# BadgerTechnologies/navigation

Measured on AMD Instinct MI355X. Metric: scored trajectories/sec (whole node) + costmap inflation cells/sec, 400x400 map, higher is better.
Workload: dtype f64

## Files before the change

### navigation_amd/csrc/planner_score.h

```cpp
#pragma once
#include "planner_common.h"

namespace navgpu {

__host__ __device__ inline size_t score_bits_bytes(int win) {
  return (((size_t)4 * win * ((win + 31) >> 5) * 4) + 15) & ~(size_t)15;
}
__host__ __device__ inline size_t score_scratch_bytes(int win) { return score_bits_bytes(win); }
__device__ __forceinline__ int divSmall(int n, int d) {
  int q = (int)((float)n * __builtin_amdgcn_rcpf((float)d));
  int r = n - q * d;
  if (r < 0) {
    --q;
    r += d;
  }
  if (r >= d) ++q;
  return q;
}

struct WorldToMapFast {
  const Geom& g;
  const double& inv_res;
  __device__ __forceinline__ bool operator()(double wx, double wy, uint32_t& mx, uint32_t& my) const {
    const double dx = wx - g.ox, dy = wy - g.oy;
    const double qx = dx * inv_res, qy = dy * inv_res;
    double fx = floor(qx), fy = floor(qy);
    const double rx = qx - fx, ry = qy - fy;
    if (__builtin_expect(fmin(rx, ry) < 1.0e-7 || fmax(rx, ry) > 1.0 - 1.0e-7, 0)) {
      fx = !(dx >= 0.0) ? -1.0 : (qx >= 1.0e6 ? 1.0e6 : (double)(int)(dx / g.res));
      fy = !(dy >= 0.0) ? -1.0 : (qy >= 1.0e6 ? 1.0e6 : (double)(int)(dy / g.res));
    }
    int ix, iy;
    asm("v_cvt_i32_f64 %0, %1" : "=v"(ix) : "v"(fx));
    asm("v_cvt_i32_f64 %0, %1" : "=v"(iy) : "v"(fy));
    mx = (uint32_t)ix;
    my = (uint32_t)iy;
    return mx < g.nx && my < g.ny;
  }
};

__device__ __forceinline__ void addCritic(double& total, bool en, double value, double scale) {
  if (!en) return;
  double cost = value;
  if (cost != 0) cost *= scale;
  total += cost;
}

constexpr uint32_t kScoreAuxBytes = 64;
__host__ __device__ inline uint32_t score_prep_reject_bytes(const PlannerDev& pl) { return (pl.max_axis * pl.max_axis + 255u) & ~255u; }
__host__ __device__ inline uint32_t score_prep_reject_offset(const PlannerDev& pl) { return pl.prep_stride - score_prep_reject_bytes(pl); }
template <size_t kAllowAbove = 48 * 1024, typename... P, typename... A>
void launchScore(void (*kernel)(P...), dim3 grid, int threads, size_t lds, hipStream_t s, A... args) {
  if (lds > kAllowAbove) hipFuncSetAttribute((const void*)kernel, hipFuncAttributeMaxDynamicSharedMemorySize, (int)lds);
  hipLaunchKernelGGL(kernel, grid, dim3(threads), lds, s, args...);
}
size_t score_table_row_bytes(const PlannerDev& pl);
size_t score_table_lds_bytes(const PlannerDev& pl);
bool score_sweep_applies(const PlannerDev& pl);
uint32_t launch_score_sweep(const PlannerDev& pl, uint32_t first, uint32_t count, hipStream_t s);
uint32_t launch_score_sweep_list(const PlannerDev& pl, const uint32_t* list, uint32_t count, hipStream_t s);

}
```

### navigation_amd/csrc/planner_score.hip

```cpp
#include "planner_score.h"

namespace navgpu {

#ifdef NAVGPU_PREP_TIMING
__device__ unsigned long long g_prep_stats[16];
#define PREP_STAMP(i) prep_t[i] = wall_clock64()
#else
#define PREP_STAMP(i)
#endif

struct ScoreRobot {
  uint32_t inst;
  Geom g;
  navgpu_robot_state st;
  const uint8_t* master;
  const uint32_t *dpath, *dgoal, *dfront;
  const int32_t* cnt;
  uint32_t nfp;
  int win, wx0, wy0;
  int win_bytes, nw;
};
__device__ __forceinline__ ScoreRobot scoreRobot(const PlannerDev& pl, uint32_t inst) {
  ScoreRobot r;
  r.inst = inst;
  r.g = geomOf(pl, inst);
  r.st = pl.state[inst];
  r.master = pl.master + (size_t)inst * pl.cells_padded;
  r.dpath = pl.path + (size_t)inst * pl.cells;
  r.dgoal = pl.goal + (size_t)inst * pl.cells;
  r.dfront = pl.goal_front + (size_t)inst * pl.cells;
  r.cnt = pl.axis_count + 4 * inst;
  r.nfp = pl.fp_n[inst];
  r.win = (int)pl.win;
  r.win_bytes = (r.win * r.win + 15) & ~15;
  r.nw = (r.win + 31) >> 5;
  return r;
}
__device__ __forceinline__ void placeWindow(ScoreRobot& r) {
  double fx = floor(((double)r.st.pos[0] - r.g.ox) / r.g.res), fy = floor(((double)r.st.pos[1] - r.g.oy) / r.g.res);
  fx = fmin(fmax(fx, -1.0e6), 1.0e6);
  fy = fmin(fmax(fy, -1.0e6), 1.0e6);
  r.wx0 = (int)fx - r.win / 2;
  r.wy0 = (int)fy - r.win / 2;
}

template <bool EXPLICIT>
__device__ __forceinline__ void stageInputs(const PlannerDev& pl, ScoreRobot& r, double* s_fp, float (*s_axis)[kMaxAxis], int* s_cnt, uint8_t* s_win) {
  const uint32_t tid = threadIdx.x;
  const Geom& g = r.g;
  if (tid < 2 * r.nfp) s_fp[tid] = pl.fp_spec[(size_t)r.inst * kMaxFootprint * 2 + tid];
  if (!EXPLICIT) {
    for (uint32_t i = tid; i < 3 * kMaxAxis; i += blockDim.x) {
      uint32_t a = i / kMaxAxis, k = i - a * kMaxAxis;
// ... 130 lines not shown
  const navgpu_robot_state& st = r.st;
  const uint32_t nfp = r.nfp;
  const int K = (int)pl.tab_steps;
  const int tnfp = (int)pl.tab_nfp;
  const int nth_s = r.cnt[2];
  const int lrows = (int)pl.tab_nth;
  double* s_trig = reinterpret_cast<double*>(s_dyn + r.win_bytes + score_bits_bytes(r.win));
  double* s_rot = s_trig + (size_t)lrows * K * 4;
  float* s_th = reinterpret_cast<float*>(s_rot + (size_t)lrows * K * tnfp * 2);
  __syncthreads();
  const double dt_t = c.sim_time / K;
  if ((int)tid < nth_s) {
    float pth = st.pos[2];
    const float vth = s_axis[2][tid];
    for (int k = 0; k < K; ++k) {
      s_th[tid * K + k] = pth;
      pth = (float)(pth + vth * dt_t);
    }
  }
  __syncthreads();
  for (int e = tid; e < nth_s * K; e += blockDim.x) {
    const double th = s_th[e];
    double sn, cs, sn2, cs2;
    sincos(th, &sn, &cs);
    sincos(M_PI_2 + th, &sn2, &cs2);
    s_trig[4 * e] = cs;
    s_trig[4 * e + 1] = sn;
    s_trig[4 * e + 2] = cs2;
    s_trig[4 * e + 3] = sn2;
    for (int v = 0; v < (int)nfp && v < tnfp; ++v) {
      const double sx = s_fp[2 * v], sy = s_fp[2 * v + 1];
      s_rot[(e * tnfp + v) * 2] = sx * cs - sy * sn;
      s_rot[(e * tnfp + v) * 2 + 1] = sx * sn + sy * cs;
    }
  }
}

__device__ __forceinline__ void storeImage(const PlannerDev& pl, const ScoreRobot& r, const uint8_t* s_dyn) {
  uint4* img = reinterpret_cast<uint4*>(pl.prep + (size_t)r.inst * pl.prep_stride);
  const uint4* lds = reinterpret_cast<const uint4*>(s_dyn);
  const uint32_t n16 = pl.prep_bytes >> 4;
  for (uint32_t i = threadIdx.x; i < n16; i += blockDim.x) img[i] = lds[i];
}

__device__ __forceinline__ void storeSweepScalars(const PlannerDev& pl, const ScoreRobot& r, const float (*s_axis)[kMaxAxis], int* s_cnt,
                                                  const uint8_t* s_dyn) {
  const uint32_t tid = threadIdx.x;
  const navgpu_dwa_config& c = pl.cfg;
  const Geom& g = r.g;
  const int32_t* cnt = r.cnt;
  const uint32_t inst = r.inst;
  const int win = r.win, wx0 = r.wx0, wy0 = r.wy0, nw = r.nw;
  const uint32_t* s_fb = reinterpret_cast<const uint32_t*>(s_dyn + r.win_bytes);
  uint8_t* rej = pl.prep + (size_t)inst * pl.prep_stride + score_prep_reject_offset(pl);
  int32_t* aux = reinterpret_cast<int32_t*>(rej - kScoreAuxBytes);
  const int c0 = win / 2;
  const uint32_t w_c0 = (uint32_t)(c0 * nw + (c0 >> 5));
  const int start_fail = ((s_fb[4 * w_c0 + 2] >> (c0 & 31)) & 1u) ? 4 : (((s_fb[4 * w_c0 + 3] >> (c0 & 31)) & 1u) ? 5 : 0);
  if (tid == 0) s_cnt[0] = (win / 2) * (win / 2);
  __syncthreads();
  {
    int dmin = win * win;
    for (int it = tid; it < win * nw; it += blockDim.x) {
      const int y = it / nw, j = it - y * nw;
      uint32_t m = (c.sum_scores ? s_fb[4 * it] : s_fb[4 * it + 1]) | (start_fail == 4 ? 0u : s_fb[4 * it + 2]) | (start_fail != 0 ? 0u : s_fb[4 * it + 3]);
      const int dy = y > c0 ? y - c0 : c0 - y;
      const int p = c0 - 32 * j;
      const uint32_t right = p <= 0 ? m : (p >= 32 ? 0u : m & (0xFFFFFFFFu << p)), left = m & ~right;
      if (right) dmin = min(dmin, (32 * j + __ffs(right) - 1 - c0) * (32 * j + __ffs(right) - 1 - c0) + dy * dy);
      if (left) dmin = min(dmin, (c0 - (32 * j + 31 - __clz(left))) * (c0 - (32 * j + 31 - __clz(left))) + dy * dy);
    }
    atomicMin(&s_cnt[0], dmin);
  }
  __syncthreads();
  if (tid == 0) {
    const double inv_res = pl.inv_res, fpd = c.forward_point_distance;
    const bool en_fwd = pl.scale_goal != 0 || (pl.align_on[inst] && pl.scale_path != 0);
    const uint32_t fwd_margin = (uint32_t)fmin(ceil(fabs(fpd) * inv_res) + 1.0, 1.0e6);
    const bool fwd_screen = !en_fwd || (2u * fwd_margin < g.nx && 2u * fwd_margin < g.ny);
    const uint32_t fwd_lo = en_fwd ? fwd_margin : 0u, fwd_nx = g.nx - 2u * fwd_lo, fwd_ny = g.ny - 2u * fwd_lo;
    const bool need_margin = !((uint32_t)wx0 - fwd_lo < fwd_nx && (uint32_t)(wx0 + win - 1) - fwd_lo < fwd_nx && (uint32_t)wy0 - fwd_lo < fwd_ny &&
                               (uint32_t)(wy0 + win - 1) - fwd_lo < fwd_ny);
    aux[0] = wx0;
    aux[1] = wy0;
    aux[2] = (int32_t)fwd_lo;
    aux[3] = (int32_t)fwd_nx;
    aux[4] = (int32_t)fwd_ny;
    aux[5] = need_margin ? 1 : 0;
    aux[6] = fwd_screen ? 1 : 0;
    aux[7] = (int)floor(sqrt((double)s_cnt[0]));
    aux[8] = start_fail;
  }
  const int nyv = max(cnt[1], 1), nxyv = cnt[0] * cnt[1];
  for (int i = tid; i < nxyv; i += blockDim.x) {
    const int ix = i / nyv, iy = i - ix * nyv;
    const double vmag = hyp2((double)s_axis[0][ix], (double)s_axis[1][iy]);
    const double eps = 1e-4;
    rej[i] = (uint8_t)(((c.min_trans_vel >= 0 && vmag + eps < c.min_trans_vel) ? 1 : 0) | ((c.max_trans_vel >= 0 && vmag - eps > c.max_trans_vel) ? 2 : 0));
  }
}

struct ScoreInputs {
  static constexpr int kAxisChunks = (3 * kMaxAxis + kScoreThreads - 1) / kScoreThreads;
  double fp;
  float axis[kAxisChunks];
};
__device__ __forceinline__ ScoreInputs loadInputs(const PlannerDev& pl, const ScoreRobot& r) {
  const uint32_t tid = threadIdx.x;
  ScoreInputs in;
  in.fp = pl.fp_spec[(size_t)r.inst * kMaxFootprint * 2 + (tid < 2 * r.nfp ? tid : 0)];
#pragma unroll
  for (int u = 0; u < ScoreInputs::kAxisChunks; ++u) {
    const uint32_t i = min(tid + (uint32_t)u * kScoreThreads, 3u * kMaxAxis - 1), a = i / kMaxAxis, k = i - a * kMaxAxis;
    in.axis[u] = pl.axis_samples[((size_t)r.inst * 3 + a) * pl.max_axis + min(k, pl.max_axis - 1)];
    if (k >= pl.max_axis) in.axis[u] = 0.f;
  }
  return in;
}
__device__ __forceinline__ void loadImage(const PlannerDev& pl, const ScoreRobot& r, const ScoreInputs& in, double* s_fp, float (*s_axis)[kMaxAxis],
                                          uint8_t* s_dyn) {
  const uint32_t tid = threadIdx.x;
  const uint4* img = reinterpret_cast<const uint4*>(pl.prep + (size_t)r.inst * pl.prep_stride);
  uint4* lds = reinterpret_cast<uint4*>(s_dyn);
  const uint32_t n16 = pl.prep_bytes >> 4;
  for (uint32_t i = tid; i < n16; i += blockDim.x) lds[i] = img[i];
  if (tid < 2 * r.nfp) s_fp[tid] = in.fp;
#pragma unroll
  for (int u = 0; u < ScoreInputs::kAxisChunks; ++u) {
    const uint32_t i = tid + (uint32_t)u * kScoreThreads;
    if (i < 3u * kMaxAxis) s_axis[i / kMaxAxis][i % kMaxAxis] = in.axis[u];
  }
  __syncthreads();
}

template <bool EXPLICIT, int CHUNK, bool AGG, bool TERMS = false, bool PROBES = false>
__device__ __forceinline__ void scoreSamples(const PlannerDev& pl, const ScoreRobot& r, const double* s_fp, const float (*s_axis)[kMaxAxis],
                                             const uint8_t* s_dyn, double* s_rc, int* s_ri, int* s_cnt, const float* explicit_sample,
                                             SampleTerms* terms = nullptr, uint32_t n_probes = 0, double* probe_cost = nullptr) {
  static_assert(!PROBES || (EXPLICIT && !TERMS), "probes are explicit samples");
  const uint32_t tid = threadIdx.x;
  const navgpu_dwa_config& c = pl.cfg;
  const Geom& g = r.g;
  const navgpu_robot_state& st = r.st;
  const uint8_t* master = r.master;
  const uint32_t *dpath = r.dpath, *dgoal = r.dgoal, *dfront = r.dfront;
  const int32_t* cnt = r.cnt;
  const uint32_t inst = r.inst, nfp = r.nfp;
  const int n_samples = PROBES ? (int)n_probes : EXPLICIT ? 1 : cnt[3];
  const int win = r.win, wx0 = r.wx0, wy0 = r.wy0, win_bytes = r.win_bytes, nw = r.nw;
  const uint8_t* s_win = s_dyn;
  const bool walk_swap = pl.cfg.allow_unknown != 0;
// ... 536 lines not shown
__global__ __launch_bounds__(kScoreThreads) void k_score_explicit_agg(PlannerDev pl, uint32_t first, const float* explicit_sample) {
  scoreExplicit<true>(pl, first, explicit_sample);
}
template <bool AGG>
__device__ __forceinline__ void checkTraj(const PlannerDev& pl, const ProbeBatch& pb) {
  extern __shared__ __align__(16) uint8_t s_dyn[];
  __shared__ double s_fp[2 * kMaxFootprint];
  __shared__ float s_axis[3][kMaxAxis];
  __shared__ int s_cnt[2];
  const uint32_t p0 = pb.offsets[blockIdx.y], n = pb.offsets[blockIdx.y + 1] - p0;
  if (blockIdx.x * kScoreThreads >= n) return;
  ScoreRobot r = scoreRobot(pl, pb.instances[blockIdx.y]);
  if (blockIdx.x == 0 && threadIdx.x == 0) pl.osc_flags[r.inst] = 0;
  stageInputs<true>(pl, r, s_fp, s_axis, s_cnt, s_dyn);
  __syncthreads();
  buildScreens(pl, r, s_dyn, reinterpret_cast<uint32_t*>(s_dyn + r.win_bytes + score_bits_bytes(r.win)));
  __syncthreads();
  scoreSamples<true, 12, AGG, false, true>(pl, r, s_fp, s_axis, s_dyn, nullptr, nullptr, s_cnt, pb.vel + 3 * (size_t)p0, nullptr, n, pb.cost + p0);
}
__global__ __launch_bounds__(kScoreThreads) void k_check_traj(PlannerDev pl, ProbeBatch pb) { checkTraj<false>(pl, pb); }
__global__ __launch_bounds__(kScoreThreads) void k_check_traj_agg(PlannerDev pl, ProbeBatch pb) { checkTraj<true>(pl, pb); }

__global__ __launch_bounds__(kScoreThreads) void k_score_terms(PlannerDev pl, uint32_t inst, SampleTerms* terms) {
  scoreGen<16, false, true>(pl, RobotRange{inst}, terms);
}
__global__ __launch_bounds__(kScoreThreads) void k_score_terms_agg(PlannerDev pl, uint32_t inst, SampleTerms* terms) {
  scoreGen<16, true, true>(pl, RobotRange{inst}, terms);
}

size_t score_window_bytes(uint32_t win) {
  return (((size_t)win * win + 15) & ~(size_t)15) + score_bits_bytes((int)win);
}
size_t score_table_row_bytes(const PlannerDev& pl) { return (size_t)pl.tab_steps * ((4 + 2 * pl.tab_nfp) * sizeof(double) + sizeof(float)); }
size_t score_table_bytes(const PlannerDev& pl) {
  return ((size_t)pl.tab_nth * score_table_row_bytes(pl) + 15) & ~(size_t)15;
}
size_t score_table_lds_bytes(const PlannerDev& pl) {
  return ((size_t)pl.tab_rows * score_table_row_bytes(pl) + 15) & ~(size_t)15;
}
uint32_t score_table_rows(const PlannerDev& pl, uint32_t win) {
  const size_t wb = score_window_bytes(win), row = score_table_row_bytes(pl);
  if (row == 0 || wb + score_table_bytes(pl) + score_scratch_bytes((int)win) > 150u * 1024u) return 0;
  for (size_t budget : {(size_t)NAVGPU_SCORE_TAB_LDS_KB * 1024, (size_t)52 * 1024, (size_t)78 * 1024}) {
    if (wb + 16 >= budget) continue;
    const size_t r = (budget - wb - 16) / row;
    if (r >= 1) return (uint32_t)std::min<size_t>(r, pl.tab_nth);
  }
  return 0;
}
size_t score_prep_bytes(const PlannerDev& pl) {
  return score_window_bytes(pl.win) + (pl.use_tables ? score_table_bytes(pl) : 0);
}
size_t score_prep_slot_bytes(const PlannerDev& pl) {
  return ((score_prep_bytes(pl) + 255) & ~(size_t)255) + kScoreAuxBytes + score_prep_reject_bytes(pl);
}
static uint32_t sweepLaunch(const PlannerDev& pl, RobotRange r, uint32_t count, hipStream_t s) { return launch_score_sweep(pl, r.first, count, s); }
static uint32_t sweepLaunch(const PlannerDev& pl, RobotList r, uint32_t count, hipStream_t s) { return launch_score_sweep_list(pl, r.list, count, s); }
template <class Robots>
static uint32_t launchScoreCycle(const PlannerDev& pl_in, Robots robots, uint32_t count, hipStream_t s) {
  PlannerDev pl = pl_in;
  const size_t win_bytes = score_window_bytes(pl.win);
  const size_t scratch = score_scratch_bytes((int)pl.win);
  if (score_sweep_applies(pl)) {
    pl.tab_bytes = (uint32_t)score_table_bytes(pl);
    pl.prep_bytes = (uint32_t)score_prep_bytes(pl);
    launchScore(k_score_prep_tab<Robots>, dim3(1, count), kScorePrepThreads, win_bytes + score_table_bytes(pl) + scratch, s, pl, robots);
    return sweepLaunch(pl, robots, count, s);
  }
  pl.use_tables = 0;
  pl.prep_bytes = (uint32_t)score_prep_bytes(pl);
  const uint32_t gen_blocks = (pl.max_samples + kScoreThreads - 1) / kScoreThreads;
  launchScore(prepGenKernel(robots), dim3(1, count), kScoreThreads, win_bytes + scratch, s, pl, robots);
  auto gen = pl.mg_generic        ? k_score_gen_agg<Robots>
             : pl.fp_chunk <= 6  ? k_score_gen<6, Robots>
             : pl.fp_chunk <= 9  ? k_score_gen<9, Robots>
             : pl.fp_chunk <= 12 ? k_score_gen<12, Robots>
                                 : k_score_gen<16, Robots>;
  launchScore(gen, dim3(gen_blocks, count), kScoreThreads, win_bytes, s, pl, robots, (const float*)nullptr);
  return gen_blocks;
}
uint32_t launch_score(const PlannerDev& pl, uint32_t first, uint32_t count, const float* explicit_sample, hipStream_t s) {
  if (explicit_sample) {
    const size_t lds = score_window_bytes(pl.win) + score_scratch_bytes((int)pl.win);
    launchScore(pl.mg_generic ? k_score_explicit_agg : k_score_explicit, dim3(1, count), kScoreThreads, lds, s, pl, first, explicit_sample);
    return 1;
  }
  return launchScoreCycle(pl, RobotRange{first}, count, s);
}
uint32_t launch_score_list(const PlannerDev& pl, const uint32_t* list, uint32_t count, hipStream_t s) { return launchScoreCycle(pl, RobotList{list}, count, s); }

void launch_check_traj(const PlannerDev& pl, const ProbeBatch& pb, uint32_t n_robots, uint32_t max_probes, hipStream_t s) {
  const size_t lds = score_window_bytes(pl.win) + score_scratch_bytes((int)pl.win);
  launchScore(pl.mg_generic ? k_check_traj_agg : k_check_traj, dim3((max_probes + kScoreThreads - 1) / kScoreThreads, n_robots), kScoreThreads, lds, s, pl, pb);
}

void launch_score_terms(const PlannerDev& pl_in, uint32_t inst, SampleTerms* terms, hipStream_t s) {
  PlannerDev pl = pl_in;
  const size_t win_bytes = score_window_bytes(pl.win);
  pl.use_tables = 0;
  pl.prep_bytes = (uint32_t)score_prep_bytes(pl);
  const uint32_t gen_blocks = (pl.max_samples + kScoreThreads - 1) / kScoreThreads;
  launchScore(k_score_prep_gen, dim3(1, 1), kScoreThreads, win_bytes + score_scratch_bytes((int)pl.win), s, pl, RobotRange{inst});
  launchScore(pl.mg_generic ? k_score_terms_agg : k_score_terms, dim3(gen_blocks, 1), kScoreThreads, win_bytes, s, pl, inst, terms);
}

#ifdef NAVGPU_PREP_TIMING
extern "C" int navgpu_debug_prep_stats(unsigned long long* out16, int reset) {
  if (out16) hipMemcpyFromSymbol(out16, HIP_SYMBOL(g_prep_stats), sizeof(unsigned long long) * 16);
  if (reset) {
    unsigned long long z[16] = {0};
    hipMemcpyToSymbol(HIP_SYMBOL(g_prep_stats), z, sizeof(z));
  }
  return 0;
}
#endif

}
```

### navigation_amd/csrc/planner_score_sweep.hip

```cpp
#include "planner_score.h"

namespace navgpu {

constexpr int kSweepThreads = NAVGPU_SCORE_TAB_THREADS;
constexpr int kSweepWaves = 6;
#ifndef NAVGPU_SWEEP_BLOCK_STEPS
#define NAVGPU_SWEEP_BLOCK_STEPS 4
#endif
#ifndef NAVGPU_SWEEP_QUEUE
#define NAVGPU_SWEEP_QUEUE 768
#endif
constexpr int kSweepBlockSteps = NAVGPU_SWEEP_BLOCK_STEPS;
constexpr int kSweepQueue = NAVGPU_SWEEP_QUEUE;
constexpr uint32_t kWalkFailed = 0x80000000u;
#ifdef NAVGPU_SWEEP_COUNTS
__device__ unsigned long long g_sweep_counts[16];
#define SW_COUNT(slot_, n_)                                                                    \
  do {                                                                                           \
    const unsigned long long swc_ = (unsigned long long)(n_);                                    \
    if ((threadIdx.x & 63u) == 0) atomicAdd(&g_sweep_counts[slot_], swc_);                       \
  } while (0)
#else
#define SW_COUNT(slot_, n_)
#endif
#ifdef NAVGPU_SWEEP_TIMING
__device__ unsigned long long g_sweep_stats[16];
#define SW_STAMP(v) const unsigned long long v = __builtin_amdgcn_s_memtime()
#define SW_ACC(i, x) sw_t[i] += (x)
#else
#define SW_STAMP(v)
#define SW_ACC(i, x)
#endif

template <int CHUNK, bool TRIGF, bool KEEP, class Robots>
__global__ __launch_bounds__(kSweepThreads, kSweepWaves) void k_score_sweep(PlannerDev pl, Robots robots) {
  constexpr int THREADS = kSweepThreads;
  extern __shared__ __align__(16) uint8_t s_dyn[];
  uint8_t* s_win = s_dyn;
  __shared__ double s_rc[THREADS / 64];
  __shared__ int s_ri[THREADS / 64];
  __shared__ int s_cnt[2];
  __shared__ float s_qx[kSweepQueue], s_qy[kSweepQueue];
  __shared__ uint32_t s_qt[kSweepQueue];
  __shared__ uint32_t s_obs[THREADS];
  __shared__ uint32_t s_qn[2];
  __shared__ uint32_t s_more[3];

  const uint32_t inst = robots(blockIdx.z);
  const uint32_t tid = threadIdx.x;
#ifdef NAVGPU_SWEEP_TIMING
  unsigned long long sw_t[10] = {0, 0, 0, 0, 0, 0, 0, 0, 0, 0};
#endif
  SW_STAMP(sw0);
  __builtin_amdgcn_s_setprio(3);
  const navgpu_dwa_config& c = pl.cfg;
  const Geom g = geomOf(pl, inst);
  const navgpu_robot_state st = pl.state[inst];
  const uint8_t* master = pl.master + (size_t)inst * pl.cells_padded;
  const uint32_t* dpath = pl.path + (size_t)inst * pl.cells;
  const uint32_t* dgoal = pl.goal + (size_t)inst * pl.cells;
  const uint32_t* dfront = pl.goal_front + (size_t)inst * pl.cells;
  const int32_t* cnt = pl.axis_count + 4 * inst;
  const int n_samples = cnt[3];
  const uint32_t nfp = pl.fp_n[inst];
  const int win = (int)pl.win;

  if (tid == 0) s_cnt[0] = s_cnt[1] = 0;
  if (tid < 2) s_qn[tid] = 0;
  if (tid < 3) s_more[tid] = 0;
  s_obs[tid] = 0;
  const uint8_t* rej_bytes = pl.prep + (size_t)inst * pl.prep_stride + score_prep_reject_offset(pl);
  const int32_t* aux = reinterpret_cast<const int32_t*>(rej_bytes - kScoreAuxBytes);
  const int wx0 = aux[0], wy0 = aux[1];
  const uint32_t fwd_lo = (uint32_t)aux[2], fwd_nx = (uint32_t)aux[3], fwd_ny = (uint32_t)aux[4];
  const bool need_margin = aux[5] != 0, fwd_screen = aux[6] != 0;
  const int free_cells = aux[7];
  const int start_fail = aux[8];
  const uint32_t osc = pl.osc_flags[inst];
  const int32_t align_on = pl.align_on[inst];
  const int win_bytes = (win * win + 15) & ~15;
  const int nw = (win + 31) >> 5;
  const bool walk_swap = pl.cfg.allow_unknown != 0;
  const uint32_t walk_fail = walk_swap ? 255u : 254u;
  const int K = (int)pl.tab_steps;
  const int tnfp = (int)pl.tab_nfp;
  const int lrows = (int)pl.tab_rows;
  double* s_trig = reinterpret_cast<double*>(s_dyn + win_bytes + score_bits_bytes(win));
  double* s_rot = s_trig + (size_t)lrows * K * 4;
  const int nxy = max(cnt[0] * cnt[1], 1);
  const uint32_t part_slot = blockIdx.y * gridDim.x + blockIdx.x;
  const int t_row_base = (int)blockIdx.y * (int)pl.tab_rows;
  const int t_rows = min(max(cnt[2] - t_row_base, 0), (int)pl.tab_rows);
  const int t_li0 = (int)blockIdx.x * THREADS;
  if (t_li0 >= t_rows * nxy) {
    if (tid == 0) {
      pl.part_cost[(size_t)inst * pl.score_blocks + part_slot] = 1.0e300;
      pl.part_index[(size_t)inst * pl.score_blocks + part_slot] = 0x7FFFFFFF;
    }
    return;
  }
  const int li = t_li0 + (int)tid;
  const int t_row = divSmall(li, nxy);
  const int t_r = li - t_row * nxy;
  const int t_ith = t_row_base + t_row;
  const bool in_range = n_samples > 0 && t_row < t_rows;
  const int sidx = t_r * cnt[2] + t_ith;
  const int nyv = max(cnt[1], 1);
  const int s_ix = divSmall(t_r, nyv), s_iy = t_r - s_ix * nyv;
  const float* axis = pl.axis_samples + (size_t)inst * 3 * pl.max_axis;
  const uint32_t amax = pl.max_axis - 1u;
  const float vs0 = axis[min((uint32_t)s_ix, amax)], vs1 = axis[pl.max_axis + min((uint32_t)s_iy, amax)], vs2 = axis[2u * pl.max_axis + min((uint32_t)t_ith, amax)];
  const uint32_t rej_xy = rej_bytes[in_range ? t_r : 0];
  auto rejected = [&]() { return !in_range || ((rej_xy & 1u) && (c.min_rot_vel >= 0 && fabs((double)vs2) + 1e-4 < c.min_rot_vel)) || (rej_xy & 2u) || K <= 0; };
  if constexpr (!KEEP) {
    if (start_fail != 0) {
      const unsigned long long m_acc = __ballot(!rejected());
      if ((tid & 63u) == 0 && m_acc != 0ull) atomicAdd(&pl.counters[2 * inst], __popcll(m_acc));
      if (tid == 0) {
        pl.part_cost[(size_t)inst * pl.score_blocks + part_slot] = 1.0e300;
        pl.part_index[(size_t)inst * pl.score_blocks + part_slot] = 0x7FFFFFFF;
      }
      return;
    }
  }
  {
    const uint4* img = reinterpret_cast<const uint4*>(pl.prep + (size_t)inst * pl.prep_stride);
    uint4* lds = reinterpret_cast<uint4*>(s_dyn);
    const int last = max(t_rows, 1) - 1;
    const int r0 = min(divSmall(t_li0, nxy), last);
    const int r1 = min(divSmall(t_li0 + THREADS - 1, nxy), last);
    const int n16w = (int)((win_bytes + score_bits_bytes(win)) >> 4);
    const int ncopy = r1 - r0 + 1;
    const int n_trig = ncopy * K * 2, n_rot = ncopy * K * tnfp;
    const int l_trig = n16w + r0 * K * 2, g_trig = n16w + (t_row_base + r0) * K * 2;
    const int l_rot = n16w + lrows * K * 2 + r0 * K * tnfp, g_rot = n16w + (int)pl.tab_nth * K * 2 + (t_row_base + r0) * K * tnfp;
    const int ia0 = (int)tid, ia1 = (int)tid + THREADS;
    const uint4 va0 = img[min(ia0, n16w - 1)], va1 = img[min(ia1, n16w - 1)];
    const uint4 vb = img[g_trig + min((int)tid, n_trig - 1)], vc = img[g_rot + min((int)tid, max(n_rot, 1) - 1)];
    if (ia0 < n16w) lds[ia0] = va0;
    if (ia1 < n16w) lds[ia1] = va1;
    if ((int)tid < n_trig) lds[l_trig + (int)tid] = vb;
    if ((int)tid < n_rot) lds[l_rot + (int)tid] = vc;
    if (n16w > 2 * THREADS || n_trig > THREADS || n_rot > THREADS) {
      for (int i = (int)tid + 2 * THREADS; i < n16w; i += THREADS) lds[i] = img[i];
      for (int i = (int)tid + THREADS; i < n_trig; i += THREADS) lds[l_trig + i] = img[g_trig + i];
      for (int i = (int)tid + THREADS; i < n_rot; i += THREADS) lds[l_rot + i] = img[g_rot + i];
    }
  }
  SW_STAMP(sw1a);
  __syncthreads();
  __builtin_amdgcn_s_setprio(0);
  SW_STAMP(sw1);
  SW_ACC(0, sw1a - sw0);
  SW_ACC(1, sw1 - sw1a);

  auto inWin = [&](int x, int y) { return (unsigned)(x - wx0) < (unsigned)win && (unsigned)(y - wy0) < (unsigned)win; };
  auto cellCost = [&](int x, int y) -> uint8_t {
    const bool in = inWin(x, y);
    uint32_t v = s_win[in ? (y - wy0) * win + (x - wx0) : 0];
    asm volatile("" : "+v"(v));
    if (walk_swap && v >= 254u) v ^= 1u;
    if (__builtin_expect(!in, 0)) v = master[y * g.nx + x];
    return (uint8_t)v;
  };
  const double inv_res = pl.inv_res;
  const WorldToMapFast w2m{g, inv_res};

  auto walkWindow = [&](const double x, const double y, const int te, uint32_t& mx, bool& outside) -> bool {
    const double* rot = s_rot + (size_t)te * tnfp * 2;
    bool off = false;
    outside = false;
    mx = 0;
    uint32_t ux, uy;
    off |= !w2m(x + rot[0], y + rot[1], ux, uy);
    const int fx0 = (int)ux, fy0 = (int)uy;
    int pxc = fx0, pyc = fy0;
    for (uint32_t v = 1; v <= nfp; ++v) {
      int vx = fx0, vy = fy0;
      if (v < nfp) {
        off |= !w2m(x + rot[2 * v], y + rot[2 * v + 1], ux, uy);
        vx = (int)ux;
        vy = (int)uy;
// ... 35 lines not shown
    w2m(x + rot[0], y + rot[1], ux, uy);
    const int fx0 = (int)ux, fy0 = (int)uy;
    int pxc = fx0, pyc = fy0;
    for (uint32_t v = 1; v <= nfp; ++v) {
      int vx = fx0, vy = fy0;
      if (v < nfp) {
        w2m(x + rot[2 * v], y + rot[2 * v + 1], ux, uy);
        vx = (int)ux;
        vy = (int)uy;
      }
      int deltax = vx - pxc, deltay = vy - pyc;
      deltax = deltax < 0 ? -deltax : deltax;
      deltay = deltay < 0 ? -deltay : deltay;
      int lx = pxc, ly = pyc;
      int xinc1, xinc2, yinc1, yinc2, den, num, numadd, numpixels;
      xinc1 = xinc2 = (vx >= pxc) ? 1 : -1;
      yinc1 = yinc2 = (vy >= pyc) ? 1 : -1;
      if (deltax >= deltay) {
        xinc1 = 0;
        yinc2 = 0;
        den = deltax;
        num = deltax / 2;
        numadd = deltay;
        numpixels = deltax;
      } else {
        xinc2 = 0;
        yinc1 = 0;
        den = deltay;
        num = deltay / 2;
        numadd = deltax;
        numpixels = deltay;
      }
      for (int cp = 0; cp <= numpixels; ++cp) {
        const uint32_t cc = master[ly * g.nx + lx];
        const uint32_t ct = (walk_swap && cc >= 254u) ? (cc ^ 1u) : cc;
        mx = ct > mx ? ct : mx;
        num += numadd;
        if (num >= den) {
          num -= den;
          lx += xinc1;
          ly += yinc1;
        }
        lx += xinc2;
        ly += yinc2;
      }
      pxc = vx;
      pyc = vy;
    }
    return mx;
  };

  double total = -1.0;
  int status = NAVGPU_SAMPLE_REJECTED;
  const float vs[3] = {vs0, vs1, vs2};
  const bool reject = rejected();
  if (in_range && !reject) status = NAVGPU_SAMPLE_SCORED;
  const double dt = pl.tab_dt;
  const double xv = vs[0], yv = vs[1], thv = vs[2];
  const bool osc_fail = ((osc & NAVGPU_OSC_FORWARD_POS_ONLY) && xv < 0.0) || ((osc & NAVGPU_OSC_FORWARD_NEG_ONLY) && xv > 0.0) ||
                        ((osc & NAVGPU_OSC_STRAFE_POS_ONLY) && yv < 0.0) || ((osc & NAVGPU_OSC_STRAFE_NEG_ONLY) && yv > 0.0) ||
                        ((osc & NAVGPU_OSC_ROT_POS_ONLY) && thv < 0.0) || ((osc & NAVGPU_OSC_ROT_NEG_ONLY) && thv > 0.0);
  const double sc_obs = pl.scale_obstacle, sc_gf = pl.scale_goal, sc_al = align_on ? pl.scale_path : 0.0, sc_path = pl.scale_path,
               sc_goal = pl.scale_goal;
  const bool en_obs = sc_obs != 0, en_gf = sc_gf != 0, en_al = sc_al != 0, en_path = sc_path != 0, en_goal = sc_goal != 0;
  int first_fail = 6;
  int fail_code = 0;
  uint32_t d_gf = 0, d_al = 0, d_path = 0, d_goal = 0;
  uint32_t fail_cell = 0xFFFFFFFFu, last_c = 0, last_f = 0xFFFFFFFFu;
  const double fpd = c.forward_point_distance;
  const uint32_t N_obst = pl.cells, N_unreach = pl.cells + 1;
  if (en_obs && nfp == 0) {
    fail_code = -9;
    first_fail = 1;
  }
  const int min_order_keep = en_obs ? 1 : en_gf ? 2 : en_al ? 3 : en_path ? 4 : en_goal ? 5 : 6;
  const int min_order = KEEP ? min_order_keep : (min_order_keep < 6 ? 5 : 6);
  uint32_t fb_off = (uint32_t)win_bytes;
  asm volatile("" : "+v"(fb_off));
  const uint4* s_fb4 = reinterpret_cast<const uint4*>(s_dyn + fb_off);
  const bool scr_sum = c.sum_scores != 0;
  const bool screen_on = fwd_screen && (nfp >= 3 || !en_obs);
  float px = st.pos[0], py = st.pos[1];
  int step = 0;
  uint32_t alive_m = (in_range && !reject && !osc_fail && first_fail > min_order) ? 0xFFFFFFFFu : 0u;
#ifdef NAVGPU_SWEEP_X_NOSTEPS
  alive_m = 0;
#endif
  const bool margin_on = __builtin_amdgcn_readfirstlane((int)need_margin) != 0;
  const uint32_t lane = tid & 63u;
  const int te0 = t_row * K;
  const double vxd = vs[0], vyd = vs[1];
  uint32_t scr_z = 0xFFFFFFFFu, scr_w = 0xFFFFFFFFu;
  const uint32_t scr_off = screen_on ? 0u : 0xFFFFFFFFu;
  SW_STAMP(sw2);
  SW_ACC(2, sw2 - sw1);
  int k_free = 0;
  {
    const float spd = sqrtf(vs0 * vs0 + vs1 * vs1) * (float)(dt * inv_res) * 1.0001f + 1.0e-4f;
    int kl = K - 1;
    if (alive_m != 0u) kl = (screen_on && !margin_on && free_cells >= 3) ? (int)fminf((float)(free_cells - 2) / spd, (float)(K - 1)) : 0;
    for (int off = 32; off > 0; off >>= 1) kl = min(kl, __shfl_xor(kl, off));
    k_free = __builtin_amdgcn_readfirstlane(kl);
  }
  for (int k = 0; k < k_free; ++k) {
    const int te = te0 + k;
    const double cs = s_trig[4 * te], sn = s_trig[4 * te + 1], cs2 = s_trig[4 * te + 2], sn2 = s_trig[4 * te + 3];
    const double tx = TRIGF ? (double)(vs[0] * (float)cs) : vxd * cs, ty = TRIGF ? (double)(vs[0] * (float)sn) : vxd * sn;
    const float nxp = (float)(px + (tx + vyd * cs2) * dt);
    const float nyp = (float)(py + (ty + vyd * sn2) * dt);
    px = nxp;
    py = nyp;
  }
  if (alive_m != 0u) step = k_free;
  SW_COUNT(9, k_free);
  SW_COUNT(10, (unsigned)k_free * (unsigned)__popcll(__ballot(alive_m != 0u)));
  if constexpr (KEEP) {
    if (k_free > 0 && start_fail != 0 && alive_m != 0u) {
      first_fail = start_fail;
      fail_code = 0;
      fail_cell = (uint32_t)(wy0 + win / 2) * g.nx + (uint32_t)(wx0 + win / 2);
      scr_z = first_fail > 4 ? 0xFFFFFFFFu : 0u;
      scr_w = 0u;
      alive_m = first_fail > min_order ? 0xFFFFFFFFu : 0u;
    }
  }
  for (uint32_t blk = 0;; ++blk) {
    SW_STAMP(sb0);
    if (__ballot(alive_m != 0u) != 0ull) {
      for (int it = 0; it < kSweepBlockSteps; ++it) {
        const int sc = min(step, K - 1);
        const int te = te0 + sc;
        const double x = px, y = py;
        const double cs = s_trig[4 * te], sn = s_trig[4 * te + 1];
        SW_COUNT(4, 1);
        SW_COUNT(8, __popcll(__ballot(alive_m != 0u)));
        const double cs2 = s_trig[4 * te + 2], sn2 = s_trig[4 * te + 3];
        const double tx = TRIGF ? (double)(vs[0] * (float)cs) : vxd * cs, ty = TRIGF ? (double)(vs[0] * (float)sn) : vxd * sn;
        const float nxp = (float)(px + (tx + vyd * cs2) * dt);
        const float nyp = (float)(py + (ty + vyd * sn2) * dt);
        uint32_t cx, cy;
        const bool ok_c = w2m(x, y, cx, cy);
        const uint32_t lx = cx - (uint32_t)wx0, ly = cy - (uint32_t)wy0;
        bool in_w = max(lx, ly) < (uint32_t)win;
        uint32_t force = (sc == K - 1) ? 0xFFFFFFFFu : scr_off;
        if (margin_on) {
          in_w = in_w && ok_c;
          if (!((cx - fwd_lo < fwd_nx) && (cy - fwd_lo < fwd_ny))) force = 0xFFFFFFFFu;
        }
        const uint32_t fb_i = in_w ? ly * (uint32_t)nw + (lx >> 5) : 0u;
        const uint4 fbw = s_fb4[fb_i];
        const uint32_t any = (scr_sum ? fbw.x : fbw.y) | (fbw.z & scr_z) | (fbw.w & scr_w) | force | (in_w ? 0u : 0xFFFFFFFFu);
        const bool unscr = ((any >> (lx & 31u)) & alive_m & 1u) != 0u;
        px = nxp;
        py = nyp;
        step -= (int)alive_m;
// ... 156 lines not shown
      if ((tid & 63u) == (uint32_t)(__ffsll((long long)__ballot(true)) - 1)) atomicAdd(&g_sweep_counts[7], 1ull);
#endif
      if (off || mx_cost >= walk_fail) {
        atomicOr(&s_obs[owner], kWalkFailed);
      } else if (tag >> 31) {
        const double f_cost = (walk_swap && mx_cost == 254u) ? 255.0 : (double)mx_cost;
        uint32_t cx, cy;
        w2m(x, y, cx, cy);
        const double occ = fmax(fmax(0.0, f_cost), (double)cellCost(cx, cy));
        atomicAdd(&s_obs[owner], (uint32_t)occ);
      }
    }
    SW_STAMP(sb3);
    SW_ACC(6, sb3 - sb2);
    __syncthreads();
    SW_STAMP(sb4);
    SW_ACC(7, sb4 - sb3);
    if ((s_obs[tid] & kWalkFailed) != 0u && first_fail > 1) {
      fail_code = -6;
      first_fail = 1;
      alive_m = 0;
    }
    if (!more) break;
  }

  {
    const bool reached = last_f != 0xFFFFFFFFu && first_fail > 1;
    const uint32_t cmax = pl.cells - 1u;
    uint32_t v_fail = 0;
    if constexpr (KEEP) v_fail = (first_fail == 4 ? dpath : dgoal)[min(fail_cell, cmax)];
    const uint32_t v_gf = dfront[min(last_f, cmax)], v_al = dpath[min(last_f, cmax)];
    const uint32_t v_path = dpath[min(last_c, cmax)], v_goal = dgoal[min(last_c, cmax)];
    if constexpr (KEEP)
      if ((first_fail == 4 || first_fail == 5) && fail_code == 0) fail_code = v_fail == N_obst ? -3 : -2;
    if (reached) {
      if (en_gf && 2 < first_fail) d_gf = v_gf;
      if (en_al && 3 < first_fail) d_al = v_al;
      if (en_path && 4 < first_fail) {
        if (v_path == N_obst || v_path == N_unreach) {
          fail_code = v_path == N_obst ? -3 : -2;
          first_fail = 4;
        } else
          d_path = v_path;
      }
      if (en_goal && 5 < first_fail) {
        if (v_goal == N_obst || v_goal == N_unreach) {
          fail_code = v_goal == N_obst ? -3 : -2;
          first_fail = 5;
        } else
          d_goal = v_goal;
      }
    }
  }
  if (in_range && !reject) {
    if (osc_fail) {
      total = -5.0;
    } else if (first_fail < 6) {
      total = KEEP ? (double)fail_code : -1.0;
    } else {
      total = 0.0;
      addCritic(total, en_obs, (double)(s_obs[tid] & ~kWalkFailed), sc_obs);
      addCritic(total, en_gf, (double)d_gf, sc_gf);
      addCritic(total, en_al, (double)d_al, sc_al);
      addCritic(total, en_path, (double)d_path, sc_path);
      addCritic(total, en_goal, (double)d_goal, sc_goal);
    }
  }
  if constexpr (KEEP) {
    if (in_range && pl.sample_cost) {
      pl.sample_cost[(size_t)inst * pl.max_samples + sidx] = total;
      pl.sample_status[(size_t)inst * pl.max_samples + sidx] = status;
    }
  }

  const bool valid = in_range && status == NAVGPU_SAMPLE_SCORED && total >= 0.0;
  double bc = valid ? total : 1.0e300;
  int bi = valid ? sidx : 0x7FFFFFFF;
  for (int off = 32; off > 0; off >>= 1) {
    double oc = __shfl_down(bc, off);
    int oi = __shfl_down(bi, off);
    if (oc < bc || (oc == bc && oi < bi)) {
      bc = oc;
      bi = oi;
    }
  }
  const unsigned long long m_scored = __ballot(in_range && status == NAVGPU_SAMPLE_SCORED);
  const unsigned long long m_valid = __ballot(valid);
  if ((tid & 63) == 0) {
    s_rc[tid >> 6] = bc;
    s_ri[tid >> 6] = bi;
    atomicAdd(&s_cnt[0], __popcll(m_scored));
    atomicAdd(&s_cnt[1], __popcll(m_valid));
  }
  __syncthreads();
  if (tid == 0) {
    for (int w = 1; w < THREADS / 64; ++w)
      if (s_rc[w] < bc || (s_rc[w] == bc && s_ri[w] < bi)) {
        bc = s_rc[w];
        bi = s_ri[w];
      }
    pl.part_cost[(size_t)inst * pl.score_blocks + part_slot] = bc;
    pl.part_index[(size_t)inst * pl.score_blocks + part_slot] = bi;
    if (s_cnt[0]) atomicAdd(&pl.counters[2 * inst], s_cnt[0]);
    if (s_cnt[1]) atomicAdd(&pl.counters[2 * inst + 1], s_cnt[1]);
  }
#ifdef NAVGPU_SWEEP_TIMING
// ... 66 lines not shown
```

Measured before the change: 6.768 billion.

## Precompute per-pair and per-row sweep records in prep; use DPP wave-min

Prep now writes 16-byte per-(vx,vy) records holding the velocities, the free-step bound and the reject and oscillation flags, plus per-rotation-row flag records. The sweep kernel reads one uint4 instead of recomputing axis loads, the hypot and sqrt, and the oscillation tests per thread. The wave minimum uses DPP plus readlane instead of shuffles, and row/column index division is replaced by a wave-uniform base with an increment loop. This adds prep work and prep-slot memory, and the float-bit min trick relies on kl values being non-negative.

```diff
diff --git a/navigation_amd/csrc/planner_score.h b/navigation_amd/csrc/planner_score.h
--- a/navigation_amd/csrc/planner_score.h
+++ b/navigation_amd/csrc/planner_score.h
@@ -47,8 +47,24 @@
 }
 
 constexpr uint32_t kScoreAuxBytes = 64;
-__host__ __device__ inline uint32_t score_prep_reject_bytes(const PlannerDev& pl) { return (pl.max_axis * pl.max_axis + 255u) & ~255u; }
-__host__ __device__ inline uint32_t score_prep_reject_offset(const PlannerDev& pl) { return pl.prep_stride - score_prep_reject_bytes(pl); }
+struct alignas(16) SweepPair {
+  float vs0, vs1;
+  float kl_pair;
+  uint32_t flags;
+};
+struct alignas(16) SweepRow {
+  double thv;
+  float vs2;
+  uint32_t flags;
+};
+static_assert(sizeof(SweepPair) == 16 && sizeof(SweepRow) == 16, "one 16-byte load per record");
+constexpr uint32_t kPairRejMin = 1u, kPairRejMax = 2u, kPairOsc = 4u;
+constexpr uint32_t kRowRejRot = 1u, kRowOsc = 2u;
+__host__ __device__ inline uint32_t score_prep_pair_bytes(const PlannerDev& pl) { return pl.max_axis * pl.max_axis * (uint32_t)sizeof(SweepPair); }
+__host__ __device__ inline uint32_t score_prep_record_bytes(const PlannerDev& pl) {
+  return (score_prep_pair_bytes(pl) + pl.max_axis * (uint32_t)sizeof(SweepRow) + 255u) & ~255u;
+}
+__host__ __device__ inline uint32_t score_prep_record_offset(const PlannerDev& pl) { return pl.prep_stride - score_prep_record_bytes(pl); }
 template <size_t kAllowAbove = 48 * 1024, typename... P, typename... A>
 void launchScore(void (*kernel)(P...), dim3 grid, int threads, size_t lds, hipStream_t s, A... args) {
   if (lds > kAllowAbove) hipFuncSetAttribute((const void*)kernel, hipFuncAttributeMaxDynamicSharedMemorySize, (int)lds);
diff --git a/navigation_amd/csrc/planner_score.hip b/navigation_amd/csrc/planner_score.hip
--- a/navigation_amd/csrc/planner_score.hip
+++ b/navigation_amd/csrc/planner_score.hip
@@ -1,4 +1,5 @@
 #include "planner_score.h"
+#include "navgpu_fleet.h"
 
 namespace navgpu {
 
@@ -235,8 +236,8 @@
   const uint32_t inst = r.inst;
   const int win = r.win, wx0 = r.wx0, wy0 = r.wy0, nw = r.nw;
   const uint32_t* s_fb = reinterpret_cast<const uint32_t*>(s_dyn + r.win_bytes);
-  uint8_t* rej = pl.prep + (size_t)inst * pl.prep_stride + score_prep_reject_offset(pl);
-  int32_t* aux = reinterpret_cast<int32_t*>(rej - kScoreAuxBytes);
+  uint8_t* rec = pl.prep + (size_t)inst * pl.prep_stride + score_prep_record_offset(pl);
+  int32_t* aux = reinterpret_cast<int32_t*>(rec - kScoreAuxBytes);
   const int c0 = win / 2;
   const uint32_t w_c0 = (uint32_t)(c0 * nw + (c0 >> 5));
   const int start_fail = ((s_fb[4 * w_c0 + 2] >> (c0 & 31)) & 1u) ? 4 : (((s_fb[4 * w_c0 + 3] >> (c0 & 31)) & 1u) ? 5 : 0);
@@ -273,13 +274,39 @@
     aux[6] = fwd_screen ? 1 : 0;
     aux[7] = (int)floor(sqrt((double)s_cnt[0]));
     aux[8] = start_fail;
-  }
+    aux[9] = (int32_t)pl.osc_flags[inst];
+  }
+  const uint32_t osc = pl.osc_flags[inst];
+  const int free_cells = (int)floor(sqrt((double)s_cnt[0]));
+  const int K = (int)pl.tab_steps;
+  const double dt = pl.tab_dt;
+  const double eps = 1e-4;
+  SweepPair* pairs = reinterpret_cast<SweepPair*>(rec);
   const int nyv = max(cnt[1], 1), nxyv = cnt[0] * cnt[1];
   for (int i = tid; i < nxyv; i += blockDim.x) {
     const int ix = i / nyv, iy = i - ix * nyv;
-    const double vmag = hyp2((double)s_axis[0][ix], (double)s_axis[1][iy]);
-    const double eps = 1e-4;
-    rej[i] = (uint8_t)(((c.min_trans_vel >= 0 && vmag + eps < c.min_trans_vel) ? 1 : 0) | ((c.max_trans_vel >= 0 && vmag - eps > c.max_trans_vel) ? 2 : 0));
+    const float vs0 = s_axis[0][ix], vs1 = s_axis[1][iy];
+    const double xv = vs0, yv = vs1;
+    const double vmag = hyp2(xv, yv);
+    const bool osc_xy = ((osc & NAVGPU_OSC_FORWARD_POS_ONLY) && xv < 0.0) || ((osc & NAVGPU_OSC_FORWARD_NEG_ONLY) && xv > 0.0) ||
+                        ((osc & NAVGPU_OSC_STRAFE_POS_ONLY) && yv < 0.0) || ((osc & NAVGPU_OSC_STRAFE_NEG_ONLY) && yv > 0.0);
+    const float spd = sqrtf(vs0 * vs0 + vs1 * vs1) * (float)(dt * pl.inv_res) * 1.0001f + 1.0e-4f;
+    SweepPair p;
+    p.vs0 = vs0;
+    p.vs1 = vs1;
+    p.kl_pair = free_cells >= 3 ? fminf((float)(free_cells - 2) / spd, (float)(K - 1)) : 0.f;
+    p.flags = ((c.min_trans_vel >= 0 && vmag + eps < c.min_trans_vel) ? kPairRejMin : 0u) | ((c.max_trans_vel >= 0 && vmag - eps > c.max_trans_vel) ? kPairRejMax : 0u) |
+              (osc_xy ? kPairOsc : 0u);
+    pairs[i] = p;
+  }
+  SweepRow* rows = reinterpret_cast<SweepRow*>(rec + score_prep_pair_bytes(pl));
+  for (int i = tid; i < cnt[2]; i += blockDim.x) {
+    SweepRow w;
+    w.vs2 = s_axis[2][i];
+    w.thv = w.vs2;
+    w.flags = ((c.min_rot_vel >= 0 && fabs((double)w.vs2) + eps < c.min_rot_vel) ? kRowRejRot : 0u) |
+              ((((osc & NAVGPU_OSC_ROT_POS_ONLY) && w.thv < 0.0) || ((osc & NAVGPU_OSC_ROT_NEG_ONLY) && w.thv > 0.0)) ? kRowOsc : 0u);
+    rows[i] = w;
   }
 }
 
@@ -922,7 +949,7 @@
   return score_window_bytes(pl.win) + (pl.use_tables ? score_table_bytes(pl) : 0);
 }
 size_t score_prep_slot_bytes(const PlannerDev& pl) {
-  return ((score_prep_bytes(pl) + 255) & ~(size_t)255) + kScoreAuxBytes + score_prep_reject_bytes(pl);
+  return ((score_prep_bytes(pl) + 255) & ~(size_t)255) + kScoreAuxBytes + score_prep_record_bytes(pl);
 }
 static uint32_t sweepLaunch(const PlannerDev& pl, RobotRange r, uint32_t count, hipStream_t s) { return launch_score_sweep(pl, r.first, count, s); }
 static uint32_t sweepLaunch(const PlannerDev& pl, RobotList r, uint32_t count, hipStream_t s) { return launch_score_sweep_list(pl, r.list, count, s); }
@@ -974,6 +1001,20 @@
   launchScore(pl.mg_generic ? k_score_terms_agg : k_score_terms, dim3(gen_blocks, 1), kScoreThreads, win_bytes, s, pl, inst, terms);
 }
 
+extern "C" int navgpu_debug_score_setup_records(navgpu_fleet* f, uint32_t inst, int32_t* aux16, void* pairs, uint32_t n_pairs, void* rows, uint32_t n_rows) {
+  if (!f || !f->rangeOk(inst, 1) || !aux16 || (n_pairs && !pairs) || (n_rows && !rows)) return NAVGPU_ERR_INVALID;
+  FleetGuard guard_(f);
+  const PlannerDev& pl = f->pl;
+  if (!f->planner_configured || !pl.prep) return NAVGPU_ERR_STATE;
+  if (n_pairs > pl.max_axis * pl.max_axis || n_rows > pl.max_axis) return NAVGPU_ERR_CAPACITY;
+  HIP_TRY(waitStream(f->stream));
+  const uint8_t* rec = pl.prep + (size_t)inst * pl.prep_stride + score_prep_record_offset(pl);
+  HIP_TRY(hipMemcpy(aux16, rec - kScoreAuxBytes, kScoreAuxBytes, hipMemcpyDeviceToHost));
+  if (n_pairs) HIP_TRY(hipMemcpy(pairs, rec, (size_t)n_pairs * sizeof(SweepPair), hipMemcpyDeviceToHost));
+  if (n_rows) HIP_TRY(hipMemcpy(rows, rec + score_prep_pair_bytes(pl), (size_t)n_rows * sizeof(SweepRow), hipMemcpyDeviceToHost));
+  return NAVGPU_OK;
+}
+
 #ifdef NAVGPU_PREP_TIMING
 extern "C" int navgpu_debug_prep_stats(unsigned long long* out16, int reset) {
   if (out16) hipMemcpyFromSymbol(out16, HIP_SYMBOL(g_prep_stats), sizeof(unsigned long long) * 16);
diff --git a/navigation_amd/csrc/planner_score_sweep.hip b/navigation_amd/csrc/planner_score_sweep.hip
--- a/navigation_amd/csrc/planner_score_sweep.hip
+++ b/navigation_amd/csrc/planner_score_sweep.hip
@@ -31,6 +31,16 @@
 #define SW_STAMP(v)
 #define SW_ACC(i, x)
 #endif
+
+__device__ __forceinline__ uint32_t waveMinU32(uint32_t v) {
+  v = min(v, (uint32_t)__builtin_amdgcn_update_dpp((int)v, (int)v, 0xB1, 0xF, 0xF, false));
+  v = min(v, (uint32_t)__builtin_amdgcn_update_dpp((int)v, (int)v, 0x4E, 0xF, 0xF, false));
+  v = min(v, (uint32_t)__builtin_amdgcn_update_dpp((int)v, (int)v, 0x141, 0xF, 0xF, false));
+  v = min(v, (uint32_t)__builtin_amdgcn_update_dpp((int)v, (int)v, 0x140, 0xF, 0xF, false));
+  const uint32_t a = (uint32_t)__builtin_amdgcn_readlane((int)v, 0), b = (uint32_t)__builtin_amdgcn_readlane((int)v, 16);
+  const uint32_t c = (uint32_t)__builtin_amdgcn_readlane((int)v, 32), d = (uint32_t)__builtin_amdgcn_readlane((int)v, 48);
+  return min(min(a, b), min(c, d));
+}
 
 template <int CHUNK, bool TRIGF, bool KEEP, class Robots>
 __global__ __launch_bounds__(kSweepThreads, kSweepWaves) void k_score_sweep(PlannerDev pl, Robots robots) {
@@ -69,15 +79,13 @@
   if (tid < 2) s_qn[tid] = 0;
   if (tid < 3) s_more[tid] = 0;
   s_obs[tid] = 0;
-  const uint8_t* rej_bytes = pl.prep + (size_t)inst * pl.prep_stride + score_prep_reject_offset(pl);
-  const int32_t* aux = reinterpret_cast<const int32_t*>(rej_bytes - kScoreAuxBytes);
+  const uint8_t* rec_bytes = pl.prep + (size_t)inst * pl.prep_stride + score_prep_record_offset(pl);
+  const int32_t* aux = reinterpret_cast<const int32_t*>(rec_bytes - kScoreAuxBytes);
   const int wx0 = aux[0], wy0 = aux[1];
   const uint32_t fwd_lo = (uint32_t)aux[2], fwd_nx = (uint32_t)aux[3], fwd_ny = (uint32_t)aux[4];
   const bool need_margin = aux[5] != 0, fwd_screen = aux[6] != 0;
-  const int free_cells = aux[7];
   const int start_fail = aux[8];
-  const uint32_t osc = pl.osc_flags[inst];
-  const int32_t align_on = pl.align_on[inst];
+  const int32_t align_on = __builtin_amdgcn_readfirstlane(pl.align_on[inst]);
   const int win_bytes = (win * win + 15) & ~15;
   const int nw = (win + 31) >> 5;
   const bool walk_swap = pl.cfg.allow_unknown != 0;
@@ -99,19 +107,21 @@
     }
     return;
   }
-  const int li = t_li0 + (int)tid;
-  const int t_row = divSmall(li, nxy);
-  const int t_r = li - t_row * nxy;
+  const int t_row0 = __builtin_amdgcn_readfirstlane(divSmall(t_li0, nxy));
+  int t_row = t_row0;
+  int t_r = t_li0 - t_row0 * nxy + (int)tid;
+  while (__ballot(t_r >= nxy) != 0ull) {
+    const bool wrap = t_r >= nxy;
+    t_r -= wrap ? nxy : 0;
+    t_row += wrap ? 1 : 0;
+  }
   const int t_ith = t_row_base + t_row;
   const bool in_range = n_samples > 0 && t_row < t_rows;
-  const int sidx = t_r * cnt[2] + t_ith;
-  const int nyv = max(cnt[1], 1);
-  const int s_ix = divSmall(t_r, nyv), s_iy = t_r - s_ix * nyv;
-  const float* axis = pl.axis_samples + (size_t)inst * 3 * pl.max_axis;
-  const uint32_t amax = pl.max_axis - 1u;
-  const float vs0 = axis[min((uint32_t)s_ix, amax)], vs1 = axis[pl.max_axis + min((uint32_t)s_iy, amax)], vs2 = axis[2u * pl.max_axis + min((uint32_t)t_ith, amax)];
-  const uint32_t rej_xy = rej_bytes[in_range ? t_r : 0];
-  auto rejected = [&]() { return !in_range || ((rej_xy & 1u) && (c.min_rot_vel >= 0 && fabs((double)vs2) + 1e-4 < c.min_rot_vel)) || (rej_xy & 2u) || K <= 0; };
+  const uint4 pair_w = reinterpret_cast<const uint4*>(rec_bytes)[in_range ? t_r : 0];
+  const uint32_t row_f = reinterpret_cast<const SweepRow*>(rec_bytes + score_prep_pair_bytes(pl))[min((uint32_t)t_ith, pl.max_axis - 1u)].flags;
+  const float vs0 = __uint_as_float(pair_w.x), vs1 = __uint_as_float(pair_w.y);
+  const uint32_t kl_pair = pair_w.z, pair_f = pair_w.w;
+  auto rejected = [&]() { return !in_range || ((pair_f & kPairRejMin) && (row_f & kRowRejRot)) || (pair_f & kPairRejMax) || K <= 0; };
   if constexpr (!KEEP) {
     if (start_fail != 0) {
       const unsigned long long m_acc = __ballot(!rejected());
@@ -127,7 +137,7 @@
     const uint4* img = reinterpret_cast<const uint4*>(pl.prep + (size_t)inst * pl.prep_stride);
     uint4* lds = reinterpret_cast<uint4*>(s_dyn);
     const int last = max(t_rows, 1) - 1;
-    const int r0 = min(divSmall(t_li0, nxy), last);
+    const int r0 = min(t_row0, last);
     const int r1 = min(divSmall(t_li0 + THREADS - 1, nxy), last);
     const int n16w = (int)((win_bytes + score_bits_bytes(win)) >> 4);
     const int ncopy = r1 - r0 + 1;
@@ -269,14 +279,11 @@
 
   double total = -1.0;
   int status = NAVGPU_SAMPLE_REJECTED;
-  const float vs[3] = {vs0, vs1, vs2};
+  const float vs[2] = {vs0, vs1};
   const bool reject = rejected();
   if (in_range && !reject) status = NAVGPU_SAMPLE_SCORED;
   const double dt = pl.tab_dt;
-  const double xv = vs[0], yv = vs[1], thv = vs[2];
-  const bool osc_fail = ((osc & NAVGPU_OSC_FORWARD_POS_ONLY) && xv < 0.0) || ((osc & NAVGPU_OSC_FORWARD_NEG_ONLY) && xv > 0.0) ||
-                        ((osc & NAVGPU_OSC_STRAFE_POS_ONLY) && yv < 0.0) || ((osc & NAVGPU_OSC_STRAFE_NEG_ONLY) && yv > 0.0) ||
-                        ((osc & NAVGPU_OSC_ROT_POS_ONLY) && thv < 0.0) || ((osc & NAVGPU_OSC_ROT_NEG_ONLY) && thv > 0.0);
+  const bool osc_fail = ((pair_f & kPairOsc) | (row_f & kRowOsc)) != 0u;
   const double sc_obs = pl.scale_obstacle, sc_gf = pl.scale_goal, sc_al = align_on ? pl.scale_path : 0.0, sc_path = pl.scale_path,
                sc_goal = pl.scale_goal;
   const bool en_obs = sc_obs != 0, en_gf = sc_gf != 0, en_al = sc_al != 0, en_path = sc_path != 0, en_goal = sc_goal != 0;
@@ -313,11 +320,9 @@
   SW_ACC(2, sw2 - sw1);
   int k_free = 0;
   {
-    const float spd = sqrtf(vs0 * vs0 + vs1 * vs1) * (float)(dt * inv_res) * 1.0001f + 1.0e-4f;
-    int kl = K - 1;
-    if (alive_m != 0u) kl = (screen_on && !margin_on && free_cells >= 3) ? (int)fminf((float)(free_cells - 2) / spd, (float)(K - 1)) : 0;
-    for (int off = 32; off > 0; off >>= 1) kl = min(kl, __shfl_xor(kl, off));
-    k_free = __builtin_amdgcn_readfirstlane(kl);
+    uint32_t kl = __float_as_uint((float)(K - 1));
+    if (alive_m != 0u) kl = (screen_on && !margin_on) ? kl_pair : 0u;
+    k_free = (int)__uint_as_float(waveMinU32(kl));
   }
   for (int k = 0; k < k_free; ++k) {
     const int te = te0 + k;
@@ -580,6 +585,9 @@
       }
     }
   }
+  int row_e = t_row;
+  asm volatile("" : "+v"(row_e));
+  const int sidx = (t_li0 + (int)tid - row_e * nxy) * cnt[2] + t_row_base + row_e;
   if (in_range && !reject) {
     if (osc_fail) {
       total = -5.0;
```

New measurement: 6.707 billion. About the same (-0.9%).
